# 1275468127/Medical-SAM2

Measured on AMD Instinct MI355X. Metric: slices/sec @1024^2 (Hiera-S), higher is better.
Workload: dtype bf16; 1 GPU; configs[1]: sam2_hiera_s 2D (train_2d SAM2 sub-sequence, forward), b=4 x 1024x1024 per GPU, 16-entry memory bank with 4 sampled memories per slice, one click per slice; forward_image -> memory_attention -> prompt encoder -> mask decoder -> memory encoder; hip_graph=True, weights=random name-keyed init

## Files before the change

### include/msam2_hip.h

```cpp
#ifndef MSAM2_HIP_H
#define MSAM2_HIP_H

#include <stddef.h>
#include <stdint.h>

#ifdef __cplusplus
extern "C" {
#endif

const char* msam2_last_error(void);

int msam2_version(void);

int msam2_operand_is_fp16(void);

int msam2_graph_begin(void* stream);

int msam2_graph_end(void* stream, void** graph_exec_out);

int msam2_graph_launch(void* graph_exec, void* stream);

int msam2_graph_destroy(void* graph_exec);

int msam2_event_create(void** ev);
// ... 47 lines not shown
int msam2_attention_kv64_dyn_fwd(const void* q, const int64_t* q_strides, const void* k, const int64_t* k_strides, const void* v, const int64_t* v_strides, void* o, const int64_t* o_strides, int64_t B, int64_t H, int64_t Lq, int64_t Lk, const void* key_count_dev, float scale, int splits, void* workspace, size_t workspace_bytes, void* stream);

int msam2_attention_kv64_dyn_partial(const void* q, const int64_t* q_strides, const void* k, const int64_t* k_strides, const void* v, const int64_t* v_strides, int64_t B, int64_t H, int64_t Lq, int64_t Lk, const void* key_count_dev, float scale, int splits, int split_begin, int split_count, void* workspace, size_t workspace_bytes, void* stream);

int msam2_window_attention_fwd(const void* q, int64_t q_token_stride, int64_t q_head_stride, int64_t hq, int64_t wq, int64_t ws_q, const void* k, const void* v, int64_t kv_token_stride, int64_t kv_head_stride, int64_t hk, int64_t wk, int64_t ws_k, const float* kpad, const float* vpad, void* o, int64_t o_token_stride, int64_t o_head_stride, int64_t B, int64_t H, int64_t D, float scale, void* stream);

int msam2_attention_small_fwd(const void* q, int64_t q_bs, int64_t q_ts, const void* k, int64_t k_bs, int64_t k_ts, const void* v, int64_t v_bs, int64_t v_ts, void* o, int64_t o_bs, int64_t o_ts, int64_t B, int64_t H, int64_t Lq, int64_t Lk, int64_t D, float scale, void* stream);

int msam2_attention_fewq_keysplit_splits(int64_t B, int64_t H);

int msam2_attention_fewq_keysplit(const void* q, int64_t q_bs, int64_t q_ts, const void* k, int64_t k_bs, int64_t k_ts, const void* v, int64_t v_bs, int64_t v_ts, float* part, int64_t B, int64_t H, int64_t Lq, int64_t Lk, int64_t D, int64_t splits, float scale, void* stream);

int msam2_window_qkv_attention_supported(int64_t dim, int64_t dim_out, int64_t heads, int64_t ws, int pool, int64_t H, int64_t W);

int msam2_window_qkv_attention_fwd(const void* xn, const void* w, const float* bias, void* o, int64_t B, int64_t H, int64_t W, int64_t dim, int64_t heads, int64_t ws, int pool, float scale, void* stream);

size_t msam2_attention_bwd_workspace_bytes(int64_t B, int64_t H, int64_t Lq, int64_t D);

int msam2_attention_bwd(const void* q, const int64_t* q_strides, const void* k, const int64_t* k_strides, const void* v, const int64_t* v_strides, const void* o, const int64_t* o_strides, const float* lse, const float* d_o, const int64_t* do_strides, float* dq, const int64_t* dq_strides, float* dk, const int64_t* dk_strides, float* dv, const int64_t* dv_strides, void* workspace, size_t workspace_bytes, int64_t B, int64_t H, int64_t Lq, int64_t Lk, int64_t D, float scale, void* stream);

int msam2_attention_bwd_dropout(const void* q, const int64_t* q_strides, const void* k, const int64_t* k_strides, const void* v, const int64_t* v_strides, const void* o, const int64_t* o_strides, const float* lse, const float* d_o, const int64_t* do_strides, float* dq, const int64_t* dq_strides, float* dk, const int64_t* dk_strides, float* dv, const int64_t* dv_strides, void* workspace, size_t workspace_bytes, int64_t B, int64_t H, int64_t Lq, int64_t Lk, int64_t D, float scale, float p, uint64_t seed, uint64_t offset, const void* seed_dev, void* stream);

int msam2_layernorm(const void* x, int in_is_16bit, int64_t ldx, const float* weight, const float* bias, void* y, int out_is_16bit, int64_t ldy, int64_t rows, int64_t C, float eps, int act, void* stream);

int msam2_layernorm_dual(const float* x, int64_t ldx, const float* weight, const float* bias, float* y, int64_t ldy, void* y16, int64_t ldy16, int64_t rows, int64_t C, float eps, void* stream);

int msam2_add_cast(const void* a, int a_is_16bit, int64_t a_s0, int64_t a_s1, const void* b, int b_is_16bit, int64_t b_s0, int64_t b_s1, float alpha, void* out, int out_is_16bit, int64_t D0, int64_t D1, int64_t C, void* stream);

int msam2_maxpool2x2(const void* x, int in_is_16bit, int64_t ldx, void* y, int out_is_16bit, int64_t ldy, int64_t B, int64_t H, int64_t W, int64_t C, void* stream);

// ... 249 lines not shown
```

### medical-sam2_amd/_lib.py

```python
from __future__ import annotations

import ctypes
import os
import subprocess

_HERE = os.path.dirname(os.path.abspath(__file__))
LIB_PATH = os.environ.get("MSAM2_LIB_PATH") or os.path.join(_HERE, "libmsam2_hip.so")

c_p = ctypes.c_void_p
c_i = ctypes.c_int
c_l = ctypes.c_int64
c_f = ctypes.c_float
c_z = ctypes.c_size_t
c_d = ctypes.c_double

SIGNATURES = {
    "msam2_version": (c_i, []),
    "msam2_last_error": (ctypes.c_char_p, []),
    "msam2_operand_is_fp16": (c_i, []),
    "msam2_gemm": (c_i, [c_p, c_l, c_p, c_l, c_p, c_p, c_p, c_l, c_i, c_l, c_p, c_l, c_i, c_l, c_l, c_l, c_i, c_p]),
    "msam2_gemm_pool2x2": (c_i, [c_p, c_l, c_p, c_l, c_p, c_p, c_l, c_l, c_l, c_l, c_l, c_l, c_p]),
    "msam2_gemm_qkv_pool2x2": (c_i, [c_p, c_l, c_p, c_l, c_p, c_p, c_l, c_p, c_l, c_l, c_l, c_l, c_l, c_l, c_l, c_p]),
    "msam2_gemm_tokens": (c_i, [c_p, c_l, c_p, c_l, c_p, c_l, c_p, c_p, c_l, c_p, c_l, c_i, c_l, c_l, c_l, c_i, c_p]),
    "msam2_gemm_rope": (c_i, [c_p, c_l, c_p, c_l, c_p, c_p, c_l, c_l, c_l, c_l, c_p, c_p, c_l, c_l, c_l, c_l, c_l, c_p]),
# ... 15 lines not shown
    "msam2_attention_workspace_bytes": (c_z, [c_l, c_l, c_l, c_l, c_i]),
    "msam2_attention_fwd": (c_i, [c_p, c_p, c_p, c_p, c_p, c_p, c_p, c_p, c_l, c_l, c_l, c_l, c_l, c_f, c_i, c_p, c_z, c_p]),
    "msam2_attention_fwd_lse": (c_i, [c_p, c_p, c_p, c_p, c_p, c_p, c_p, c_p, c_l, c_l, c_l, c_l, c_l, c_f, c_i, c_p, c_z, c_p, c_p]),
    "msam2_attention_fwd_lse_dropout": (c_i, [c_p, c_p, c_p, c_p, c_p, c_p, c_p, c_p, c_l, c_l, c_l, c_l, c_l, c_f, c_i, c_p, c_z, c_p, c_f,
                                              ctypes.c_uint64, ctypes.c_uint64, c_p, c_p]),
    "msam2_attention_kv64_fwd": (c_i, [c_p, c_p, c_p, c_p, c_p, c_p, c_p, c_p, c_l, c_l, c_l, c_l, c_f, c_i, c_p, c_z, c_p]),
    "msam2_attention_kv64_partial": (c_i, [c_p, c_p, c_p, c_p, c_p, c_p, c_l, c_l, c_l, c_l, c_f, c_i, c_i, c_i, c_p, c_z, c_p]),
    "msam2_attention_kv64_dyn_fwd": (c_i, [c_p, c_p, c_p, c_p, c_p, c_p, c_p, c_p, c_l, c_l, c_l, c_l, c_p, c_f, c_i, c_p, c_z, c_p]),
    "msam2_attention_kv64_dyn_partial": (c_i, [c_p, c_p, c_p, c_p, c_p, c_p, c_l, c_l, c_l, c_l, c_p, c_f, c_i, c_i, c_i, c_p, c_z, c_p]),
    "msam2_attention_effective_splits": (c_i, [c_l, c_i]),
    "msam2_attention_merge": (c_i, [c_p, c_p, c_l, c_l, c_l, c_l, c_l, c_i, c_p, c_z, c_p]),
    "msam2_window_attention_fwd": (c_i, [c_p, c_l, c_l, c_l, c_l, c_l, c_p, c_p, c_l, c_l, c_l, c_l, c_l, c_p, c_p, c_p, c_l, c_l,
                                         c_l, c_l, c_l, c_f, c_p]),
    "msam2_window_qkv_attention_supported": (c_i, [c_l, c_l, c_l, c_l, c_i, c_l, c_l]),
    "msam2_window_qkv_attention_fwd": (c_i, [c_p, c_p, c_p, c_p, c_l, c_l, c_l, c_l, c_l, c_l, c_i, c_f, c_p]),
    "msam2_attention_small_fwd": (c_i, [c_p, c_l, c_l, c_p, c_l, c_l, c_p, c_l, c_l, c_p, c_l, c_l, c_l, c_l, c_l, c_l, c_l, c_f,
                                        c_p]),
    "msam2_add_cast": (c_i, [c_p, c_i, c_l, c_l, c_p, c_i, c_l, c_l, c_f, c_p, c_i, c_l, c_l, c_l, c_p]),
    "msam2_maxpool2x2": (c_i, [c_p, c_i, c_l, c_p, c_i, c_l, c_l, c_l, c_l, c_l, c_p]),
    "msam2_upsample2x_add": (c_i, [c_p, c_p, c_l, c_l, c_l, c_l, c_p]),
    "msam2_rope_table": (c_i, [c_p, c_p, c_l, c_l, c_f, c_p]),
    "msam2_rope_inplace": (c_i, [c_p, c_l, c_l, c_l, c_l, c_l, c_l, c_l, c_p, c_p, c_p]),
    "msam2_bilinear_upsample": (c_i, [c_p, c_p, c_l, c_l, c_l, c_l, c_l, c_p]),
    "msam2_sine_pos_2d": (c_i, [c_p, c_l, c_l, c_l, c_f, c_p]),
    "msam2_fourier_pe_grid": (c_i, [c_p, c_p, c_l, c_l, c_l, c_p]),
    "msam2_hiera_pos_embed": (c_i, [c_p, c_p, c_p, c_l, c_l, c_l, c_l, c_l, c_l, c_p]),
    "msam2_im2col_patch7x7s4": (c_i, [c_p, c_p, c_l, c_l, c_p]),
    "msam2_patch_embed7x7s4": (c_i, [c_p, c_p, c_p, c_p, c_p, c_l, c_l, c_l, c_p]),
    "msam2_im2col3x3s2": (c_i, [c_p, c_p, c_l, c_l, c_l, c_l, c_l, c_p]),
    "msam2_conv3x3s2_ln_gelu": (c_i, [c_p, c_i, c_p, c_p, c_p, c_p, c_p, c_l, c_l, c_l, c_l, c_l, c_i, c_f, c_f, c_p]),
# ... 159 lines not shown
```

### medical-sam2_amd/csrc/attention.hip

```cpp
#include "common.h"
#ifdef MSAM2_STAMP
__device__ unsigned long long g_stamp[16];
__device__ unsigned long long g_wgtime[4096][4];
#define STAMP(var)                                                                     \
  do {                                                                                 \
    __builtin_amdgcn_sched_barrier(0);                                                 \
    asm volatile("s_memtime %0\n\ts_waitcnt lgkmcnt(0)" : "=s"(var)::"memory");         \
    __builtin_amdgcn_sched_barrier(0);                                                 \
  } while (0)
#define STAMP_DECL unsigned long long t0_ = 0, t1_ = 0, t2_ = 0, t3_ = 0, t4_ = 0, t5_ = 0, acc_[5] = {0, 0, 0, 0, 0}
#else
#define STAMP(var)
#define STAMP_DECL
#endif
#include <stdlib.h>
#include <type_traits>

#ifndef MSAM2_RESCALE_SLACK
#define MSAM2_RESCALE_SLACK 8.f
#endif

struct AttnParams {
  const op16 *q, *k, *v;
  op16* o;
  int64_t q_bs, q_hs, q_ts, k_bs, k_hs, k_ts, v_bs, v_hs, v_ts, o_bs, o_hs, o_ts;
  int B, H, Lq, Lk;
  float scale_log2;
  int win, ws_q, ws_k, hq, wq, hk, wk, nwy, nwx;
  const float *kpad, *vpad;
  int splits;
  int defer_merge;
  int split_begin, split_cnt;
  const int* lk_dev;
  op16* o_part;
  float* ml_part;
// ... 7 lines not shown
  static constexpr int KS = D * 2 + 16;
  static constexpr int VS = D * 2 + (((D * 2) % 128 == 64) ? 0 : 64);
  static constexpr int STAGE = BK * (KS + VS);
  static constexpr int LDS_BYTES = 2 * STAGE;
};


struct WgCoords {
  int x, y, z;
};
__device__ __forceinline__ WgCoords xcd_wg_coords() {
  const int gx = gridDim.x, gy = gridDim.y;
  const int nwg = gx * gy * gridDim.z;
  const int lid = xcd_tile_order(blockIdx.x + gx * (blockIdx.y + gy * blockIdx.z), nwg);
  return {lid % gx, (lid / gx) % gy, lid / (gx * gy)};
}

template <int DBLK>
__device__ __forceinline__ void softmax_move_reference(float mx, float& m_run, float& l_run, f32x16 (&o)[DBLK]) {
  const float m_new = fmaxf(m_run, mx);
  if (__any(m_new > m_run + MSAM2_RESCALE_SLACK)) {
    const float alpha = (m_run == -INFINITY) ? 0.f : __builtin_amdgcn_exp2f(m_run - m_new);
    l_run *= alpha;
#pragma unroll
    for (int d = 0; d < DBLK; ++d)
#pragma unroll
      for (int e = 0; e < 16; ++e) o[d][e] *= alpha;
    m_run = m_new;
  }
}

__device__ __forceinline__ int64_t win_token_offset(int t, int ws, int wy, int wx, int himg, int wimg, bool& valid) {
  const int ty = t / ws, tx = t - ty * ws;
  const int y = wy * ws + ty, x = wx * ws + tx;
  valid = (y < himg) && (x < wimg);
  return (int64_t)y * wimg + x;
}

template <int D, int NW, bool WIN>
__global__ __launch_bounds__(NW * 64, (WIN && NW == 4) ? 3 : 1) void attn_fwd_kernel(AttnParams p) {
  using C = AttnCfg<D>;
  constexpr int NT = NW * 64;
  constexpr int DSTEPS = D / 16;
  constexpr int DBLK = D / 32;
// ... 1551 lines not shown
  ws1_ = __builtin_amdgcn_s_memrealtime();
#endif
  if (wave * 32 >= p.Lq) return;

  f32x16 o[DBLK];
#pragma unroll
  for (int d = 0; d < DBLK; ++d)
#pragma unroll
    for (int e = 0; e < 16; ++e) o[d][e] = 0.f;
  float m_run = -INFINITY, l_run = 0.f;
  const int li = lane & 15;
  const int v_off = (4 * h + (li >> 2)) * RB + (16 * ((lane >> 4) & 1) + 4 * (li & 3)) * 2;
  const int ntiles = (p.Lk + BK - 1) / BK, nfull = p.Lk / BK;
  auto tile_step = [&](int tile, auto masked_tag) __attribute__((always_inline)) {
    constexpr bool MASKED = decltype(masked_tag)::value;
    const int key0 = tile * BK;
    const int krow = key0 + r;
    const unsigned char* kp = ksm + krow * RB;
    const int kx = (krow >> 2) & 3;
    f32x16 s;
#pragma unroll
    for (int e = 0; e < 16; ++e) s[e] = 0.f;
#pragma unroll
    for (int st = 0; st < DSTEPS; ++st) {
      const int c = 2 * st + h;
      const op16x8 kf = *reinterpret_cast<const op16x8*>(kp + (((c & ~3) | ((c & 3) ^ kx)) << 4));
      s = MSAM2_MFMA_32x32x16(kf, qf[st], s, 0, 0, 0);
    }
    float mx = -INFINITY;
#pragma unroll
    for (int e = 0; e < 16; ++e) {
      if constexpr (MASKED) {
        if (key0 + s_frag_key(e, h) >= p.Lk) s[e] = -INFINITY;
      }
      mx = fmaxf(mx, s[e]);
    }
    mx = half_max(mx) * p.scale_log2;
    softmax_move_reference(mx, m_run, l_run, o);
    float psum = 0.f;
    op16x8 pf[2];
    const float nm = -m_run;
#pragma unroll
    for (int e = 0; e < 16; ++e) {
      const float pe = __builtin_amdgcn_exp2f(__builtin_fmaf(s[e], p.scale_log2, nm));
      psum += pe;
      pf[e >> 3][e & 7] = f2op_fast(pe);
    }
    l_run += psum;
    const int nv = MASKED ? min(BK, lk8 - key0) : BK;
#pragma unroll
    for (int d = 0; d < DBLK; ++d) {
#pragma unroll
      for (int st = 0; st < 2; ++st) {
        const unsigned char* a0 = vsm + (key0 + 16 * st) * RB + v_off + d * 64;
        short4_t lo = {0, 0, 0, 0}, hi = {0, 0, 0, 0};
        if (!MASKED || 16 * st < nv) lo = __builtin_amdgcn_ds_read_tr16_b64_v4i16((short4_t __attribute__((address_space(3)))*)(a0));
        if (!MASKED || 16 * st + 8 < nv) hi = __builtin_amdgcn_ds_read_tr16_b64_v4i16((short4_t __attribute__((address_space(3)))*)(a0 + 8 * RB));
        short8_t vv8;
        vv8[0] = lo[0]; vv8[1] = lo[1]; vv8[2] = lo[2]; vv8[3] = lo[3];
        vv8[4] = hi[0]; vv8[5] = hi[1]; vv8[6] = hi[2]; vv8[7] = hi[3];
        o[d] = MSAM2_MFMA_32x32x16(__builtin_bit_cast(op16x8, vv8), pf[st], o[d], 0, 0, 0);
      }
    }
  };
  for (int tile = 0; tile < nfull; ++tile) tile_step(tile, std::false_type{});
  if (nfull < ntiles) tile_step(nfull, std::true_type{});
  const float l_tot = half_sum(l_run);
#ifdef MSAM2_STAMP
  ws2_ = __builtin_amdgcn_s_memrealtime();
#endif
  const float inv = 1.f / l_tot;
  if (qvalid) ATTN_STORE_O_ROWS(DBLK, p.o + (int64_t)b * p.o_bs + (int64_t)head * p.o_hs + qtok * p.o_ts, o, inv, h);
#ifdef MSAM2_STAMP
  wait_vmcnt<0>();
  ws3_ = __builtin_amdgcn_s_memrealtime();
  if (tid == 0) {
    const int wg = blockIdx.x + gridDim.x * blockIdx.y;
    if (wg < 4096) { g_wgtime[wg][0] = ws0_; g_wgtime[wg][1] = ws1_; g_wgtime[wg][2] = ws2_; g_wgtime[wg][3] = ws3_; }
// ... 679 lines not shown
```

### medical-sam2_amd/csrc/attn_winproj.hip

```cpp
#include "common.h"
#include <stdlib.h>

struct WinProjParams {
  const op16* xn;
  const op16* w;
  const float* bias;
  op16* o;
  int heads, H, W, nwx, nw;
  int n_units;
  float scale_log2;
};

__device__ __forceinline__ float quad_max(float v) {
  const int a = __builtin_amdgcn_mov_dpp(__builtin_bit_cast(int, v), 0xB1, 0xF, 0xF, true);
  v = fmaxf(v, __builtin_bit_cast(float, a));
  const int b = __builtin_amdgcn_mov_dpp(__builtin_bit_cast(int, v), 0x4E, 0xF, 0xF, true);
  return fmaxf(v, __builtin_bit_cast(float, b));
}

template <int DIM, int NB, bool QUADMAX>
__device__ __forceinline__ void winproj_T(const unsigned char* slab, const float* bias, const op16x8 (&xf)[NB][DIM / 16], int r, int h,
                                          op16x8 (&out)[NB][3][2]) {
  constexpr int KS = DIM / 16, RB = DIM * 2;
#pragma unroll
// ... 187 lines not shown
          f32x16 o[1];
#pragma unroll
          for (int e = 0; e < 16; ++e) o[0][e] = 0.f;
#pragma unroll
          for (int kb = 0; kb < NB; ++kb)
#pragma unroll
            for (int st = 0; st < 2; ++st) o[0] = MSAM2_MFMA_32x32x16(vf[kb][st], pf[qb][kb][st], o[0], 0, 0, 0);
          if (do_store) ATTN_STORE_O_ROWS(1, p.o + otok[qb] * (heads * D) + head * D + db * 32, o, inv[qb], h);
        }
      }
    }
  }
#endif
}

extern "C" int msam2_window_qkv_attention_supported(int64_t dim, int64_t dim_out, int64_t heads, int64_t ws, int pool, int64_t H,
                                                    int64_t W) {
  if (heads <= 0 || dim_out != heads * 96 || H <= 0 || W <= 0) return 0;
  if (!(ws == 8 || ws == 4) || H % ws || W % ws) return 0;
  if (pool && (H % 2 || W % 2)) return 0;
  if (ws == 4 && ((H / 4) * (W / 4)) % 2) return 0;
  if (dim == 96) return ws == 8 && heads <= 2;
  if (dim == 192) return ws == 4 && heads <= 8;
  return 0;
}

template <int DIM, int WS, bool POOL, bool STREAM>
static int launch_winproj(const WinProjParams& p, hipStream_t s) {
  constexpr int NWV = 8, SLAB = 96 * DIM * 2;
  const int lds = (STREAM ? 2 : 3 * p.heads) * SLAB + 3 * p.heads * 96 * 4;
  ensure_dyn_lds<attn_winproj_kernel<DIM, WS, POOL, STREAM, NWV>>(160 * 1024);
  const int n_pass = (p.n_units + NWV - 1) / NWV;
  hipLaunchKernelGGL((attn_winproj_kernel<DIM, WS, POOL, STREAM, NWV>), dim3((unsigned)min(256, n_pass)), dim3(NWV * 64), lds, s, p);
  return msam2_check_launch("window_qkv_attention_fwd");
}

extern "C" int msam2_window_qkv_attention_fwd(const void* xn, const void* w, const float* bias, void* o, int64_t B, int64_t H, int64_t W,
                                              int64_t dim, int64_t heads, int64_t ws, int pool, float scale, void* stream) {
  MSAM2_REQUIRE(xn && w && bias && o, "window_qkv_attention: null tensor");
  MSAM2_REQUIRE(B > 0 && H > 0 && W > 0 && heads > 0, "window_qkv_attention: empty problem");
  MSAM2_REQUIRE(msam2_window_qkv_attention_supported(dim, heads * 96, heads, ws, pool, H, W),
                "window_qkv_attention: dim %lld, %lld heads, window %lld, pool %d on %lld x %lld tokens is not built", (long long)dim,
                (long long)heads, (long long)ws, pool, (long long)H, (long long)W);
  MSAM2_REQUIRE((((uintptr_t)xn | (uintptr_t)w | (uintptr_t)bias) & 15) == 0 && ((uintptr_t)o & 7) == 0, "window_qkv_attention: 16-byte aligned tensors");
  MSAM2_REQUIRE(scale > 0.f, "window_qkv_attention: scale must be positive");
  const int64_t nw = (H / ws) * (W / ws), units = ws == 8 ? B * nw : B * nw / 2;
  MSAM2_REQUIRE(B * nw < (1ll << 30), "window_qkv_attention: too many windows");
  WinProjParams p = {(const op16*)xn, (const op16*)w, bias, (op16*)o, (int)heads, (int)H, (int)W, (int)(W / ws), (int)nw, (int)units,
                     scale * 1.4426950408889634f};
  hipStream_t s = (hipStream_t)stream;
  if (dim == 96) return pool ? launch_winproj<96, 8, true, false>(p, s) : launch_winproj<96, 8, false, false>(p, s);
  return pool ? launch_winproj<192, 4, true, true>(p, s) : launch_winproj<192, 4, false, true>(p, s);
}
```

### medical-sam2_amd/csrc/common.h

```cpp
#pragma once
#include <hip/hip_runtime.h>
#include <stdint.h>

#if defined(MSAM2_OPERAND_BF16)
typedef __bf16 op16;
#define MSAM2_OPERAND_IS_FP16 0
#define MSAM2_MFMA_32x32x16 __builtin_amdgcn_mfma_f32_32x32x16_bf16
#else
typedef _Float16 op16;
#define MSAM2_OPERAND_IS_FP16 1
#define MSAM2_MFMA_32x32x16 __builtin_amdgcn_mfma_f32_32x32x16_f16
#endif
typedef __attribute__((ext_vector_type(8))) op16 op16x8;
typedef __attribute__((ext_vector_type(4))) op16 op16x4;
typedef __attribute__((ext_vector_type(2))) op16 op16x2;
typedef __attribute__((ext_vector_type(4))) short short4_t;
typedef __attribute__((ext_vector_type(8))) short short8_t;
typedef __attribute__((ext_vector_type(16))) float f32x16;
typedef __attribute__((ext_vector_type(4))) float f32x4;

#define MSAM2_OK 0
#define MSAM2_ERR_ARG -1
#define MSAM2_ERR_LAUNCH -2

// ... 137 lines not shown
template <int ROW_BYTES_>
struct DmaImage {
  static constexpr int ROW_BYTES = ROW_BYTES_;
  static_assert(ROW_BYTES == 128 || ROW_BYTES == 64, "two images exist: 128-byte rows, slot c ^ ((r >> 1) & 7); 64-byte rows, c ^ ((r >> 2) & 3)");
  static constexpr int CPR = ROW_BYTES / 16;
  static constexpr int PIECE_ROWS = 1024 / ROW_BYTES;
  __device__ __forceinline__ static int swz(int r) { return (r >> (ROW_BYTES == 128 ? 1 : 2)) & (CPR - 1); }
  __device__ __forceinline__ static int piece_row(int piece, int lane) { return piece * PIECE_ROWS + (lane >> (ROW_BYTES == 128 ? 3 : 2)); }
  __device__ __forceinline__ static int src_chunk(int r, int lane) { return (lane & (CPR - 1)) ^ swz(r); }
};
typedef DmaImage<128> Img128;
typedef DmaImage<64> Img64;

template <int RB>
__device__ __forceinline__ int mlp_swz(int c, int r) {
  if constexpr (RB == 192) return (c & ~3) | ((c & 3) ^ ((r >> 2) & 3));
  else return (c & ~7) | ((c & 7) ^ ((r >> 1) & 7));
}

__device__ __forceinline__ constexpr int s_frag_key(int e, int h) { return (e & 3) + 8 * (e >> 2) + 4 * h; }

#define ATTN_STORE_O_ROWS(DBLK, dst, o, inv, h)                                           \
  do {                                                                                \
    op16* const dst_ = (dst);                                                         \
    _Pragma("unroll") for (int d_ = 0; d_ < DBLK; ++d_)                               \
      _Pragma("unroll") for (int g_ = 0; g_ < 4; ++g_) {                              \
        op16x4 w_;                                                                    \
        _Pragma("unroll") for (int e_ = 0; e_ < 4; ++e_) w_[e_] = f2op((o)[d_][4 * g_ + e_] * (inv)); \
        *reinterpret_cast<op16x4*>(dst_ + d_ * 32 + 8 * g_ + 4 * (h)) = w_;           \
      }                                                                               \
  } while (0)
// ... 280 lines not shown
```

### medical-sam2_amd/modeling/encoder.py

```python
from __future__ import annotations

from typing import List, Optional, Tuple

import torch
import torch.nn as nn

from .. import ops
from .common import OP16, F32, WeightCache, nchw_view, to_bf16, tokens_of, v_f32, w_bf16
from .position import PositionEmbeddingSine


import os as _os
_POOL_GEMM = _os.environ.get("MSAM2_NO_POOL_GEMM") is None
_QPOOL_GEMM = _os.environ.get("MSAM2_NO_QPOOL_GEMM") is None
_FUSED_MLP = _os.environ.get("MSAM2_NO_FUSED_MLP") is None
_FUSED_QKV_ATTN = _os.environ.get("MSAM2_NO_FUSED_QKV_ATTN") is None
_FUSED_PATCH = _os.environ.get("MSAM2_NO_FUSED_PATCH") is None
_FUSED_GEMM_LN = _os.environ.get("MSAM2_NO_FUSED_GEMM_LN") is None
_FUSED_GEMM_LN_K = frozenset(int(k) for k in _os.environ.get("MSAM2_FUSED_GEMM_LN_K", "384,1536").split(",") if k.strip())
_FUSED_MLP_LN = _os.environ.get("MSAM2_NO_FUSED_MLP_LN") is None
_FUSED_MLP_LN_MIN_TOKENS = 1024
_FUSED_PROJ_MLP = _os.environ.get("MSAM2_NO_FUSED_PROJ_MLP") is None
_FUSED_PROJ_MLP_DIMS = frozenset(int(k) for k in _os.environ.get("MSAM2_FUSED_PROJ_MLP_DIMS", "96,192").split(",") if k.strip())
_FUSED_PROJ_MLP_NEXT_LN_DIMS = frozenset(int(k) for k in _os.environ.get("MSAM2_FUSED_PROJ_MLP_NEXT_LN_DIMS", "").split(",") if k.strip())
_TWO_LAUNCH = 0


class two_launch_qkv_attention:

    def __enter__(self):
        global _TWO_LAUNCH
# ... 188 lines not shown
        scale = 1.0 / (D ** 0.5)
        if xn is None:
            xn = ops.layernorm(t, v_f32(wc, "n1w", self.norm1.weight), v_f32(wc, "n1b", self.norm1.bias), 1e-6)
        pool = self.q_stride is not None
        if self.dim != dim_out:
            if _POOL_GEMM and pool and B * H * W >= 256 and H % 2 == 0 and W % 2 == 0:
                shortcut = ops.gemm_pool2x2(xn, w_bf16(wc, "pw", self.proj.weight), v_f32(wc, "pb", self.proj.bias), B, H, W)
            else:
                shortcut = ops.gemm(xn, w_bf16(wc, "pw", self.proj.weight), v_f32(wc, "pb", self.proj.bias), out_dtype=F32)
                if pool:
                    shortcut = ops.maxpool2x2(shortcut, B, H, W)
        else:
            shortcut = t
        Hq, Wq = (H // 2, W // 2) if pool else (H, W)
        attn_in_one_kernel = (fused_qkv_attn and _FUSED_QKV_ATTN and self.window_size > 0 and Dp == D
                              and ops.window_qkv_attention_supported(self.dim, dim_out, heads, self.window_size, pool, H, W))
        if attn_in_one_kernel:
            o = ops.window_qkv_attention(xn, qkv_w, qkv_b, B, H, W, heads, self.window_size, pool, scale)
        else:
            if _POOL_GEMM and _QPOOL_GEMM and pool and B * H * W >= 256 and H % 2 == 0 and W % 2 == 0 and width % 32 == 0:
                qkv, qp = ops.gemm_qkv_pool2x2(xn, qkv_w, qkv_b, B, H, W, width)
            else:
                qkv = ops.gemm(xn, qkv_w, qkv_b)
                qp = ops.maxpool2x2(qkv[:, :width], B, H, W) if pool else None
            if self.window_size > 0:
                o = ops.window_attention(qkv, B, H, W, heads, self.window_size, qkv_b, q_pooled=qp, scale=scale)
            else:
                v5 = qkv.view(B, H * W, 3, heads, Dp)
                q = (qp.view(B, Hq * Wq, heads, Dp) if pool else v5[:, :, 0]).permute(0, 2, 1, 3)
                o = ops.attention(q, v5[:, :, 1].permute(0, 2, 1, 3), v5[:, :, 2].permute(0, 2, 1, 3), scale=scale)
# ... 176 lines not shown
```

### medical-sam2_amd/ops.py

```python
from __future__ import annotations

import ctypes
import math
from typing import Optional, Tuple

import torch

from ._lib import check, lib

OP16 = torch.float16 if lib().msam2_operand_is_fp16() else torch.bfloat16

F32 = torch.float32
ACT_NONE, ACT_GELU, ACT_RELU, ACT_SIGMOID = 0, 1, 2, 3


def _stream() -> int:
    return torch.cuda.current_stream().cuda_stream


def _p(t: Optional[torch.Tensor]):
    return None if t is None else t.data_ptr()


def _is_bf16(t: torch.Tensor) -> int:
# ... 461 lines not shown
def window_qkv_attention_supported(dim: int, dim_out: int, heads: int, ws: int, pool: bool, H: int, W: int) -> bool:
    return bool(lib().msam2_window_qkv_attention_supported(dim, dim_out, heads, ws, int(bool(pool)), H, W))


def window_qkv_attention(xn: torch.Tensor, w: torch.Tensor, bias: torch.Tensor, B: int, H: int, W: int, heads: int, ws: int,
                         pool: bool = False, scale: Optional[float] = None) -> torch.Tensor:
    _req(xn.dim() == 2 and w.dim() == 2 and xn.shape[0] == B * H * W and xn.shape[1] == w.shape[1] and w.shape[0] == 3 * heads * 96,
         "window_qkv_attention shapes")
    _req(xn.dtype == OP16 and w.dtype == OP16 and xn.is_contiguous() and w.is_contiguous(), "window_qkv_attention operands: 16-bit, contiguous")
    _req(bias.dtype == F32 and bias.is_contiguous() and bias.numel() == w.shape[0], "window_qkv_attention: bias is fp32 [3*heads*96]")
    hq, wq = (H // 2, W // 2) if pool else (H, W)
    o = torch.empty(B * hq * wq, heads * 96, dtype=OP16, device=xn.device)
    check(lib().msam2_window_qkv_attention_fwd(_p(xn), _p(w), _p(bias), _p(o), B, H, W, xn.shape[1], heads, ws, int(bool(pool)),
                                               scale if scale is not None else 1.0 / math.sqrt(96), _stream()))
    return o


def attention_small(q: torch.Tensor, k: torch.Tensor, v: torch.Tensor, heads: int, out: Optional[torch.Tensor] = None) -> torch.Tensor:
    B, Lq, C = q.shape
    Lk = k.shape[1]
    D = C // heads
    for t in (q, k, v):
        _req(t.dtype == OP16 and t.stride(2) == 1, "attention_small tensors must be 16-bit (ops.OP16), channel-contiguous")
    o = out if out is not None else torch.empty(B, Lq, C, dtype=OP16, device=q.device)
    _req(o.dtype == OP16 and o.shape == (B, Lq, C) and o.stride(2) == 1, "attention_small: out is 16-bit [B,Lq,C] with contiguous channels")
    check(lib().msam2_attention_small_fwd(_p(q), q.stride(0), q.stride(1), _p(k), k.stride(0), k.stride(1), _p(v), v.stride(0),
                                          v.stride(1), _p(o), o.stride(0), o.stride(1), B, heads, Lq, Lk, D,
                                          1.0 / math.sqrt(D), _stream()))
    return o

# ... 1233 lines not shown
```

Before: 793.1 slices/s.

## Fuse QKV projection and 14x14 window attention for dim-384 Hiera stage

Adds a fused kernel for the dim-384, 4-head, window-14 Hiera stage. It streams QKV weight pieces through double-buffered LDS, projects K/V/Q per window and head, and runs flash-style attention in the same kernel, so the QKV tensor is never written to global memory. Work units are ordered by cost and include partial edge windows, whose padded keys are filled with the bias values. The shared tile step is moved into a macro header, and the encoder enables the path by default when H*W >= 1024. The trade-off is recomputing K/V projections per head inside a one-block-per-CU kernel with large LDS use, which limits occupancy.

```diff
diff --git a/include/msam2_hip.h b/include/msam2_hip.h
--- a/include/msam2_hip.h
+++ b/include/msam2_hip.h
@@ -85,6 +85,8 @@
 int msam2_window_qkv_attention_supported(int64_t dim, int64_t dim_out, int64_t heads, int64_t ws, int pool, int64_t H, int64_t W);
 
 int msam2_window_qkv_attention_fwd(const void* xn, const void* w, const float* bias, void* o, int64_t B, int64_t H, int64_t W, int64_t dim, int64_t heads, int64_t ws, int pool, float scale, void* stream);
+
+int msam2_window_qkv_attention_units(int64_t B, int64_t H, int64_t W, int64_t heads, int32_t* out, int64_t cap);
 
 size_t msam2_attention_bwd_workspace_bytes(int64_t B, int64_t H, int64_t Lq, int64_t D);
 
diff --git a/medical-sam2_amd/_lib.py b/medical-sam2_amd/_lib.py
--- a/medical-sam2_amd/_lib.py
+++ b/medical-sam2_amd/_lib.py
@@ -53,6 +53,7 @@
                                          c_l, c_l, c_l, c_f, c_p]),
     "msam2_window_qkv_attention_supported": (c_i, [c_l, c_l, c_l, c_l, c_i, c_l, c_l]),
     "msam2_window_qkv_attention_fwd": (c_i, [c_p, c_p, c_p, c_p, c_l, c_l, c_l, c_l, c_l, c_l, c_i, c_f, c_p]),
+    "msam2_window_qkv_attention_units": (c_i, [c_l, c_l, c_l, c_l, c_p, c_l]),
     "msam2_attention_small_fwd": (c_i, [c_p, c_l, c_l, c_p, c_l, c_l, c_p, c_l, c_l, c_p, c_l, c_l, c_l, c_l, c_l, c_l, c_l, c_f,
                                         c_p]),
     "msam2_add_cast": (c_i, [c_p, c_i, c_l, c_l, c_p, c_i, c_l, c_l, c_f, c_p, c_i, c_l, c_l, c_l, c_p]),
diff --git a/medical-sam2_amd/csrc/attention.hip b/medical-sam2_amd/csrc/attention.hip
--- a/medical-sam2_amd/csrc/attention.hip
+++ b/medical-sam2_amd/csrc/attention.hip
@@ -16,9 +16,7 @@
 #include <stdlib.h>
 #include <type_traits>
 
-#ifndef MSAM2_RESCALE_SLACK
-#define MSAM2_RESCALE_SLACK 8.f
-#endif
+#include "attn_wintile.h"
 
 struct AttnParams {
   const op16 *q, *k, *v;
@@ -56,20 +54,6 @@
   const int nwg = gx * gy * gridDim.z;
   const int lid = xcd_tile_order(blockIdx.x + gx * (blockIdx.y + gy * blockIdx.z), nwg);
   return {lid % gx, (lid / gx) % gy, lid / (gx * gy)};
-}
-
-template <int DBLK>
-__device__ __forceinline__ void softmax_move_reference(float mx, float& m_run, float& l_run, f32x16 (&o)[DBLK]) {
-  const float m_new = fmaxf(m_run, mx);
-  if (__any(m_new > m_run + MSAM2_RESCALE_SLACK)) {
-    const float alpha = (m_run == -INFINITY) ? 0.f : __builtin_amdgcn_exp2f(m_run - m_new);
-    l_run *= alpha;
-#pragma unroll
-    for (int d = 0; d < DBLK; ++d)
-#pragma unroll
-      for (int e = 0; e < 16; ++e) o[d][e] *= alpha;
-    m_run = m_new;
-  }
 }
 
 __device__ __forceinline__ int64_t win_token_offset(int t, int ws, int wy, int wx, int himg, int wimg, bool& valid) {
@@ -1651,54 +1635,7 @@
   const int ntiles = (p.Lk + BK - 1) / BK, nfull = p.Lk / BK;
   auto tile_step = [&](int tile, auto masked_tag) __attribute__((always_inline)) {
     constexpr bool MASKED = decltype(masked_tag)::value;
-    const int key0 = tile * BK;
-    const int krow = key0 + r;
-    const unsigned char* kp = ksm + krow * RB;
-    const int kx = (krow >> 2) & 3;
-    f32x16 s;
-#pragma unroll
-    for (int e = 0; e < 16; ++e) s[e] = 0.f;
-#pragma unroll
-    for (int st = 0; st < DSTEPS; ++st) {
-      const int c = 2 * st + h;
-      const op16x8 kf = *reinterpret_cast<const op16x8*>(kp + (((c & ~3) | ((c & 3) ^ kx)) << 4));
-      s = MSAM2_MFMA_32x32x16(kf, qf[st], s, 0, 0, 0);
-    }
-    float mx = -INFINITY;
-#pragma unroll
-    for (int e = 0; e < 16; ++e) {
-      if constexpr (MASKED) {
-        if (key0 + s_frag_key(e, h) >= p.Lk) s[e] = -INFINITY;
-      }
-      mx = fmaxf(mx, s[e]);
-    }
-    mx = half_max(mx) * p.scale_log2;
-    softmax_move_reference(mx, m_run, l_run, o);
-    float psum = 0.f;
-    op16x8 pf[2];
-    const float nm = -m_run;
-#pragma unroll
-    for (int e = 0; e < 16; ++e) {
-      const float pe = __builtin_amdgcn_exp2f(__builtin_fmaf(s[e], p.scale_log2, nm));
-      psum += pe;
-      pf[e >> 3][e & 7] = f2op_fast(pe);
-    }
-    l_run += psum;
-    const int nv = MASKED ? min(BK, lk8 - key0) : BK;
-#pragma unroll
-    for (int d = 0; d < DBLK; ++d) {
-#pragma unroll
-      for (int st = 0; st < 2; ++st) {
-        const unsigned char* a0 = vsm + (key0 + 16 * st) * RB + v_off + d * 64;
-        short4_t lo = {0, 0, 0, 0}, hi = {0, 0, 0, 0};
-        if (!MASKED || 16 * st < nv) lo = __builtin_amdgcn_ds_read_tr16_b64_v4i16((short4_t __attribute__((address_space(3)))*)(a0));
-        if (!MASKED || 16 * st + 8 < nv) hi = __builtin_amdgcn_ds_read_tr16_b64_v4i16((short4_t __attribute__((address_space(3)))*)(a0 + 8 * RB));
-        short8_t vv8;
-        vv8[0] = lo[0]; vv8[1] = lo[1]; vv8[2] = lo[2]; vv8[3] = lo[3];
-        vv8[4] = hi[0]; vv8[5] = hi[1]; vv8[6] = hi[2]; vv8[7] = hi[3];
-        o[d] = MSAM2_MFMA_32x32x16(__builtin_bit_cast(op16x8, vv8), pf[st], o[d], 0, 0, 0);
-      }
-    }
+    ATTN_WIN_TILE_STEP(tile, MASKED, p.Lk, p.scale_log2);
   };
   for (int tile = 0; tile < nfull; ++tile) tile_step(tile, std::false_type{});
   if (nfull < ntiles) tile_step(nfull, std::true_type{});
diff --git a/medical-sam2_amd/csrc/attn_winproj.hip b/medical-sam2_amd/csrc/attn_winproj.hip
--- a/medical-sam2_amd/csrc/attn_winproj.hip
+++ b/medical-sam2_amd/csrc/attn_winproj.hip
@@ -1,4 +1,5 @@
 #include "common.h"
+#include "attn_wintile.h"
 #include <stdlib.h>
 
 struct WinProjParams {
@@ -225,9 +226,249 @@
 #endif
 }
 
+struct Win384Units {
+  int B, H, W, heads;
+  int fy, fx, ry, rx;
+  int kind[4], win[4], end[4];
+  int n_units;
+};
+
+struct Win384Unit {
+  int b, wy, wx, head, vh, vw;
+};
+
+static inline Win384Units win384_units(int64_t B, int64_t H, int64_t W, int64_t heads) {
+  Win384Units u = {};
+  u.B = (int)B; u.H = (int)H; u.W = (int)W; u.heads = (int)heads;
+  u.fy = (int)(H / 14); u.fx = (int)(W / 14); u.ry = (int)(H % 14); u.rx = (int)(W % 14);
+  const int win[4] = {u.fy * u.fx, u.rx ? u.fy : 0, u.ry ? u.fx : 0, (u.rx && u.ry) ? 1 : 0};
+  const int tok[4] = {196, 14 * u.rx, 14 * u.ry, u.ry * u.rx};
+  int order[4] = {0, 1, 2, 3};
+  auto cost = [&](int k) { return win[k] ? (tok[k] + 31) / 32 : 0; };
+  for (int i = 1; i < 4; ++i)
+    for (int j = i; j > 0 && cost(order[j]) > cost(order[j - 1]); --j) { const int t = order[j]; order[j] = order[j - 1]; order[j - 1] = t; }
+  int run = 0;
+  for (int c = 0; c < 4; ++c) {
+    u.kind[c] = order[c]; u.win[c] = win[order[c]];
+    run += u.B * u.win[c] * u.heads;
+    u.end[c] = run;
+  }
+  u.n_units = run;
+  return u;
+}
+
+__host__ __device__ __forceinline__ Win384Unit win384_unit(const Win384Units& u, int j) {
+  int c = 0;
+  while (c < 3 && j >= u.end[c]) ++c;
+  if (c) j -= u.end[c - 1];
+  const int kind = u.kind[c], nw = u.win[c];
+  const int wi = j % nw, b = (j / nw) % u.B, head = j / (nw * u.B);
+  switch (kind) {
+    case 0: return {b, wi / u.fx, wi % u.fx, head, 14, 14};
+    case 1: return {b, wi, u.fx, head, 14, u.rx};
+    case 2: return {b, u.fy, wi, head, u.ry, 14};
+    default: return {b, u.fy, u.fx, head, u.ry, u.rx};
+  }
+}
+
+struct Win384Params {
+  const op16* xn;
+  const op16* w;
+  const float* bias;
+  op16* o;
+  Win384Units u;
+  float scale_log2;
+};
+
+#ifndef WIN384_AG
+#define WIN384_AG 4
+#endif
+constexpr int WIN384_WAVES = 7, WIN384_PIECE_BYTES = 32 * 768, WIN384_LK = 196, WIN384_LK8 = 200;
+constexpr int WIN384_LDS = 2 * WIN384_PIECE_BYTES + (WIN384_LK + WIN384_LK8) * 192 + 3 * 4 * 96 * 4;
+
+__global__ __launch_bounds__(WIN384_WAVES * 64, 1) void attn_winproj384_kernel(Win384Params p) {
+#if defined(__HIP_DEVICE_COMPILE__)
+  constexpr int D = 96, DIM = 384, KS = DIM / 16, WRB = DIM * 2, CPR = DIM / 8, HEADS = 4, WS = 14, NWV = WIN384_WAVES;
+  constexpr int RB = D * 2, DSTEPS = D / 16, DBLK = D / 32, BK = 32, LK = WIN384_LK, lk8 = WIN384_LK8;
+  constexpr int AG = WIN384_AG, PIECE = WIN384_PIECE_BYTES, DMAS = PIECE / 1024, PW = (DMAS + NWV - 1) / NWV, STEPS = 9;
+  extern __shared__ __attribute__((aligned(1024))) unsigned char smem[];
+  unsigned char* const ksm = smem + 2 * PIECE;
+  unsigned char* const vsm = ksm + LK * RB;
+  float* const bsm = reinterpret_cast<float*>(vsm + lk8 * RB);
+  const int tid = threadIdx.x;
+  const int wave = __builtin_amdgcn_readfirstlane(tid >> 6), lane = tid & 63;
+  const int r = lane & 31, h = lane >> 5;
+  for (int i = tid; i < 3 * HEADS * D; i += NWV * 64) bsm[i] = p.bias[i];
+  if (tid < (lk8 - LK) * RB / 16) *reinterpret_cast<uint4*>(vsm + LK * RB + tid * 16) = make_uint4(0, 0, 0, 0);
+
+  const auto w_rsrc = raw_rsrc(p.w, 3 * HEADS * D * WRB);
+  unsigned off[PW];
+#pragma unroll
+  for (int j = 0; j < PW; ++j) {
+    const int f = min(j * NWV + wave, DMAS - 1) * 64 + lane, row = f / CPR, c = f % CPR;
+    off[j] = (unsigned)(row * WRB + mlp_swz<WRB>(c, row) * 16);
+  }
+  auto issue = [&](int head, int s, int slot) {
+    const unsigned soff = (unsigned)((((s / 3 == 2 ? 0 : s / 3 + 1) * HEADS + head) * D + (s % 3) * 32) * WRB);
+    unsigned char* d = smem + slot * PIECE;
+#pragma unroll
+    for (int j = 0; j < PW; ++j)
+      if (j * NWV + wave < DMAS) glds16_asm(w_rsrc, d + (j * NWV + wave) * 1024, off[j], soff);
+  };
+
+  const int n_units = p.u.n_units;
+  issue(win384_unit(p.u, blockIdx.x).head, 0, 0);
+  __syncthreads();
+  int g_step = 0;
+  const int swap_r = (r & ~12) | ((r & 4) << 1) | ((r & 8) >> 1);
+  auto chunk_offsets = [&](int row, int (&aoff)[8]) {
+#pragma unroll
+    for (int k = 0; k < 8; ++k) aoff[k] = mlp_swz<WRB>(2 * k + h, row) << 4;
+  };
+  const int li = lane & 15;
+  const int v_off = (4 * h + (li >> 2)) * RB + (16 * ((lane >> 4) & 1) + 4 * (li & 3)) * 2;
+
+#pragma unroll 1
+  for (int j = blockIdx.x; j < n_units; j += gridDim.x) {
+    const Win384Unit un = win384_unit(p.u, j);
+    const int head = un.head, nvalid = un.vh * un.vw;
+    const int jn = j + (int)gridDim.x;
+    const int next_head = jn < n_units ? win384_unit(p.u, jn).head : -1;
+    auto piece_ptr = [&](int s) -> const unsigned char* {
+      const int slot = g_step & 1;
+      wait_vmcnt<0>();
+      __syncthreads();
+      if (s + 1 < STEPS) issue(head, s + 1, slot ^ 1);
+      else if (next_head >= 0) issue(next_head, 0, slot ^ 1);
+      ++g_step;
+      return smem + slot * PIECE;
+    };
+
+    const bool wave_on = wave * 32 < nvalid;
+    const int v = wave * 32 + r;
+    const bool valid = v < nvalid;
+    const int vc = min(v, nvalid - 1), ty = vc / un.vw, tx = vc - ty * un.vw;
+    const int key = ty * WS + tx;
+    const int64_t tok = ((int64_t)un.b * p.u.H + un.wy * WS + ty) * p.u.W + un.wx * WS + tx;
+    auto pad_rows = [&]() {
+      for (int c = tid; c < LK * (RB / 16); c += NWV * 64) {
+        const int pk = c / (RB / 16), cc = c - pk * (RB / 16), py = pk / WS, px = pk - py * WS;
+        if (py >= un.vh || px >= un.vw) {
+          op16x8 a, bb;
+#pragma unroll
+          for (int e = 0; e < 8; ++e) {
+            a[e] = f2op(bsm[(HEADS + head) * D + cc * 8 + e]);
+            bb[e] = f2op(bsm[(2 * HEADS + head) * D + cc * 8 + e]);
+          }
+          *reinterpret_cast<op16x8*>(ksm + pk * RB + (((cc & ~3) | ((cc & 3) ^ ((pk >> 2) & 3))) << 4)) = a;
+          *reinterpret_cast<op16x8*>(vsm + pk * RB + (cc << 4)) = bb;
+        }
+      }
+    };
+    if (!wave_on) {
+#pragma unroll 1
+      for (int s = 0; s < STEPS; ++s) {
+        piece_ptr(s);
+        if (s == 0 && nvalid < LK) pad_rows();
+      }
+      continue;
+    }
+    op16x8 xf[KS];
+    {
+      const op16* xr = p.xn + tok * DIM;
+#pragma unroll
+      for (int k = 0; k < KS; ++k) xf[k] = __builtin_bit_cast(op16x8, *reinterpret_cast<const uint4*>(xr + 16 * k + 8 * h));
+    }
+    auto project = [&](const unsigned char* pc, int row, const int (&aoff)[8]) -> f32x16 {
+      const unsigned char* pr = pc + row * WRB;
+      f32x16 acc;
+#pragma unroll
+      for (int e = 0; e < 16; ++e) acc[e] = 0.f;
+      op16x8 a[2][AG];
+#pragma unroll
+      for (int i = 0; i < AG; ++i) a[0][i] = *reinterpret_cast<const op16x8*>(pr + aoff[i]);
+#pragma unroll
+      for (int g = 0; g < KS / AG; ++g) {
+        if (g + 1 < KS / AG) {
+#pragma unroll
+          for (int i = 0; i < AG; ++i) {
+            const int k = AG * (g + 1) + i;
+            a[(g + 1) & 1][i] = *reinterpret_cast<const op16x8*>(pr + aoff[k & 7] + 256 * (k >> 3));
+          }
+        }
+#pragma unroll
+        for (int i = 0; i < AG; ++i) acc = MSAM2_MFMA_32x32x16(a[g & 1][i], xf[AG * g + i], acc, 0, 0, 0);
+        __builtin_amdgcn_sched_barrier(0);
+      }
+      return acc;
+    };
+
+    int aoff_k[8];
+    chunk_offsets(r, aoff_k);
+#pragma unroll 1
+    for (int s = 0; s < 6; ++s) {
+      const int isv = s / 3, db = s % 3;
+      const unsigned char* pc = piece_ptr(s);
+      if (s == 0 && nvalid < LK) pad_rows();
+      {
+        const f32x16 acc = project(pc, r, aoff_k);
+        const float* bp = bsm + ((1 + isv) * HEADS + head) * D + db * 32 + 4 * h;
+        if (valid) {
+#pragma unroll
+          for (int g = 0; g < 4; ++g) {
+            const f32x4 bv = *reinterpret_cast<const f32x4*>(bp + 8 * g);
+            op16x4 w4;
+#pragma unroll
+            for (int e = 0; e < 4; ++e) w4[e] = f2op(acc[4 * g + e] + bv[e]);
+            const int cc = 4 * db + g;
+            if (isv) *reinterpret_cast<op16x4*>(vsm + key * RB + (cc << 4) + 8 * h) = w4;
+            else *reinterpret_cast<op16x4*>(ksm + key * RB + (((cc & ~3) | ((cc & 3) ^ ((key >> 2) & 3))) << 4) + 8 * h) = w4;
+          }
+        }
+      }
+    }
+    op16x8 qf[DSTEPS];
+    const unsigned qmask = valid ? 0xffffffffu : 0u;
+    int aoff_q[8];
+    chunk_offsets(swap_r, aoff_q);
+#pragma unroll
+    for (int db = 0; db < DBLK; ++db) {
+      const unsigned char* pc = piece_ptr(6 + db);
+      {
+        const f32x16 acc = project(pc, swap_r, aoff_q);
+        const float* bp = bsm + head * D + db * 32 + 8 * h;
+#pragma unroll
+        for (int st = 0; st < 2; ++st) {
+          const f32x4 b0 = *reinterpret_cast<const f32x4*>(bp + 16 * st), b1 = *reinterpret_cast<const f32x4*>(bp + 16 * st + 4);
+#pragma unroll
+          for (int e = 0; e < 4; ++e) {
+            qf[2 * db + st][e] = f2op(acc[8 * st + e] + b0[e]);
+            qf[2 * db + st][4 + e] = f2op(acc[8 * st + 4 + e] + b1[e]);
+          }
+          uint4 qu = __builtin_bit_cast(uint4, qf[2 * db + st]);
+          qu.x &= qmask; qu.y &= qmask; qu.z &= qmask; qu.w &= qmask;
+          qf[2 * db + st] = __builtin_bit_cast(op16x8, qu);
+        }
+      }
+    }
+
+    __builtin_amdgcn_sched_barrier(0);
+    f32x16 o[DBLK];
+    zero_acc(o);
+    float m_run = -INFINITY, l_run = 0.f;
+#pragma unroll 1
+    for (int tile = 0; tile < LK / BK; ++tile) ATTN_WIN_TILE_STEP(tile, false, LK, p.scale_log2);
+    ATTN_WIN_TILE_STEP(LK / BK, true, LK, p.scale_log2);
+    const float inv = 1.f / half_sum(l_run);
+    if (valid) ATTN_STORE_O_ROWS(DBLK, p.o + tok * (HEADS * D) + head * D, o, inv, h);
+  }
+#endif
+}
+
 extern "C" int msam2_window_qkv_attention_supported(int64_t dim, int64_t dim_out, int64_t heads, int64_t ws, int pool, int64_t H,
                                                     int64_t W) {
   if (heads <= 0 || dim_out != heads * 96 || H <= 0 || W <= 0) return 0;
+  if (ws == 14) return dim == 384 && heads == 4 && !pool;
   if (!(ws == 8 || ws == 4) || H % ws || W % ws) return 0;
   if (pool && (H % 2 || W % 2)) return 0;
   if (ws == 4 && ((H / 4) * (W / 4)) % 2) return 0;
@@ -255,11 +496,31 @@
                 (long long)heads, (long long)ws, pool, (long long)H, (long long)W);
   MSAM2_REQUIRE((((uintptr_t)xn | (uintptr_t)w | (uintptr_t)bias) & 15) == 0 && ((uintptr_t)o & 7) == 0, "window_qkv_attention: 16-byte aligned tensors");
   MSAM2_REQUIRE(scale > 0.f, "window_qkv_attention: scale must be positive");
+  hipStream_t s = (hipStream_t)stream;
+  if (ws == 14) {
+    MSAM2_REQUIRE(B * ((H + 13) / 14) * ((W + 13) / 14) * heads < (1ll << 30) && B * H * W < (1ll << 31), "window_qkv_attention: too many windows");
+    Win384Params q = {(const op16*)xn, (const op16*)w, bias, (op16*)o, win384_units(B, H, W, heads), scale * 1.4426950408889634f};
+    ensure_dyn_lds<attn_winproj384_kernel>(160 * 1024);
+    hipLaunchKernelGGL(attn_winproj384_kernel, dim3((unsigned)min(256, q.u.n_units)), dim3(WIN384_WAVES * 64), WIN384_LDS, s, q);
+    return msam2_check_launch("window_qkv_attention_fwd(384)");
+  }
   const int64_t nw = (H / ws) * (W / ws), units = ws == 8 ? B * nw : B * nw / 2;
   MSAM2_REQUIRE(B * nw < (1ll << 30), "window_qkv_attention: too many windows");
   WinProjParams p = {(const op16*)xn, (const op16*)w, bias, (op16*)o, (int)heads, (int)H, (int)W, (int)(W / ws), (int)nw, (int)units,
                      scale * 1.4426950408889634f};
-  hipStream_t s = (hipStream_t)stream;
   if (dim == 96) return pool ? launch_winproj<96, 8, true, false>(p, s) : launch_winproj<96, 8, false, false>(p, s);
   return pool ? launch_winproj<192, 4, true, true>(p, s) : launch_winproj<192, 4, false, true>(p, s);
 }
+
+extern "C" int msam2_window_qkv_attention_units(int64_t B, int64_t H, int64_t W, int64_t heads, int32_t* out, int64_t cap) {
+  MSAM2_REQUIRE(B > 0 && msam2_window_qkv_attention_supported(heads * 96, heads * 96, heads, 14, 0, H, W), "window_qkv_attention_units: form not built");
+  MSAM2_REQUIRE(B * ((H + 13) / 14) * ((W + 13) / 14) * heads < (1ll << 30), "window_qkv_attention_units: too many windows");
+  MSAM2_REQUIRE(cap >= 0 && (out || cap == 0), "window_qkv_attention_units: null list");
+  const Win384Units u = win384_units(B, H, W, heads);
+  for (int j = 0; j < u.n_units && j < cap; ++j) {
+    const Win384Unit un = win384_unit(u, j);
+    const int row[5] = {un.b, un.wy, un.wx, un.head, (un.vh * un.vw + 31) / 32};
+    for (int i = 0; i < 5; ++i) out[5 * j + i] = row[i];
+  }
+  return u.n_units;
+}
diff --git a/medical-sam2_amd/csrc/attn_wintile.h b/medical-sam2_amd/csrc/attn_wintile.h
--- /dev/null
+++ b/medical-sam2_amd/csrc/attn_wintile.h
@@ -0,0 +1,67 @@
+#pragma once
+#include "common.h"
+
+#ifndef MSAM2_RESCALE_SLACK
+#define MSAM2_RESCALE_SLACK 8.f
+#endif
+
+template <int DBLK>
+__device__ __forceinline__ void softmax_move_reference(float mx, float& m_run, float& l_run, f32x16 (&o)[DBLK]) {
+  const float m_new = fmaxf(m_run, mx);
+  if (__any(m_new > m_run + MSAM2_RESCALE_SLACK)) {
+    const float alpha = (m_run == -INFINITY) ? 0.f : __builtin_amdgcn_exp2f(m_run - m_new);
+    l_run *= alpha;
+#pragma unroll
+    for (int d = 0; d < DBLK; ++d)
+#pragma unroll
+      for (int e = 0; e < 16; ++e) o[d][e] *= alpha;
+    m_run = m_new;
+  }
+}
+
+#define ATTN_WIN_TILE_STEP(tile, MASKED, Lk, scale_log2)                                                                                  \
+  do {                                                                                                                                    \
+    const int key0 = (tile) * BK;                                                                                                         \
+    const int krow = key0 + r;                                \
+    const unsigned char* kp = ksm + krow * RB;                                                                                            \
+    const int kx = (krow >> 2) & 3;                                                                                                       \
+    f32x16 s;                                                                                                                             \
+    _Pragma("unroll") for (int e = 0; e < 16; ++e) s[e] = 0.f;                                                                            \
+    _Pragma("unroll") for (int st = 0; st < DSTEPS; ++st) {                                                                               \
+      const int c = 2 * st + h;                                                                                                           \
+      const op16x8 kf = *reinterpret_cast<const op16x8*>(kp + (((c & ~3) | ((c & 3) ^ kx)) << 4));                                        \
+      s = MSAM2_MFMA_32x32x16(kf, qf[st], s, 0, 0, 0);                                                                                    \
+    }                                                                                                                                     \
+    float mx = -INFINITY;                                                                                                                 \
+    _Pragma("unroll") for (int e = 0; e < 16; ++e) {                                                                                      \
+      if constexpr (MASKED) {                                                                                                             \
+        if (key0 + s_frag_key(e, h) >= (Lk)) s[e] = -INFINITY;                                                                            \
+      }                                                                                                                                   \
+      mx = fmaxf(mx, s[e]);                                                                                                               \
+    }                                                                                                                                     \
+    mx = half_max(mx) * (scale_log2);                                                                \
+    softmax_move_reference(mx, m_run, l_run, o);                                                                                          \
+    float psum = 0.f;                                                                                                                     \
+    op16x8 pf[2];                                                                                                                         \
+    const float nm = -m_run;                                                                 \
+    _Pragma("unroll") for (int e = 0; e < 16; ++e) {                                                                                      \
+      const float pe = __builtin_amdgcn_exp2f(__builtin_fmaf(s[e], (scale_log2), nm));                                                    \
+      psum += pe;                                                                                                                         \
+      pf[e >> 3][e & 7] = f2op_fast(pe);                                                                                                  \
+    }                                                                                                                                     \
+    l_run += psum;                                                                                                                        \
+    const int nv = MASKED ? min(BK, lk8 - key0) : BK;                          \
+    _Pragma("unroll") for (int d = 0; d < DBLK; ++d) {                                                                                    \
+      _Pragma("unroll") for (int st = 0; st < 2; ++st) {                                                                                  \
+                         \
+        const unsigned char* a0 = vsm + (key0 + 16 * st) * RB + v_off + d * 64;                                                           \
+        short4_t lo = {0, 0, 0, 0}, hi = {0, 0, 0, 0};                                                                                    \
+        if (!MASKED || 16 * st < nv) lo = __builtin_amdgcn_ds_read_tr16_b64_v4i16((short4_t __attribute__((address_space(3)))*)(a0));     \
+        if (!MASKED || 16 * st + 8 < nv) hi = __builtin_amdgcn_ds_read_tr16_b64_v4i16((short4_t __attribute__((address_space(3)))*)(a0 + 8 * RB)); \
+        short8_t vv8;                                                                                                                     \
+        vv8[0] = lo[0]; vv8[1] = lo[1]; vv8[2] = lo[2]; vv8[3] = lo[3];                                                                   \
+        vv8[4] = hi[0]; vv8[5] = hi[1]; vv8[6] = hi[2]; vv8[7] = hi[3];                                                                   \
+        o[d] = MSAM2_MFMA_32x32x16(__builtin_bit_cast(op16x8, vv8), pf[st], o[d], 0, 0, 0);                                               \
+      }                                                                                                                                   \
+    }                                                                                                                                     \
+  } while (0)
diff --git a/medical-sam2_amd/csrc/common.h b/medical-sam2_amd/csrc/common.h
--- a/medical-sam2_amd/csrc/common.h
+++ b/medical-sam2_amd/csrc/common.h
@@ -175,7 +175,8 @@
 
 template <int RB>
 __device__ __forceinline__ int mlp_swz(int c, int r) {
-  if constexpr (RB == 192) return (c & ~3) | ((c & 3) ^ ((r >> 2) & 3));
+  if constexpr (RB == 768) return c ^ (r & 15);
+  else if constexpr (RB == 192) return (c & ~3) | ((c & 3) ^ ((r >> 2) & 3));
   else return (c & ~7) | ((c & 7) ^ ((r >> 1) & 7));
 }
 
diff --git a/medical-sam2_amd/modeling/encoder.py b/medical-sam2_amd/modeling/encoder.py
--- a/medical-sam2_amd/modeling/encoder.py
+++ b/medical-sam2_amd/modeling/encoder.py
@@ -15,6 +15,8 @@
 _QPOOL_GEMM = _os.environ.get("MSAM2_NO_QPOOL_GEMM") is None
 _FUSED_MLP = _os.environ.get("MSAM2_NO_FUSED_MLP") is None
 _FUSED_QKV_ATTN = _os.environ.get("MSAM2_NO_FUSED_QKV_ATTN") is None
+_FUSED_QKV_ATTN_384 = _os.environ.get("MSAM2_NO_FUSED_QKV_ATTN_384") is None
+_FUSED_QKV_ATTN_384_MIN_TOKENS = 1024
 _FUSED_PATCH = _os.environ.get("MSAM2_NO_FUSED_PATCH") is None
 _FUSED_GEMM_LN = _os.environ.get("MSAM2_NO_FUSED_GEMM_LN") is None
 _FUSED_GEMM_LN_K = frozenset(int(k) for k in _os.environ.get("MSAM2_FUSED_GEMM_LN_K", "384,1536").split(",") if k.strip())
@@ -233,6 +235,7 @@
             shortcut = t
         Hq, Wq = (H // 2, W // 2) if pool else (H, W)
         attn_in_one_kernel = (fused_qkv_attn and _FUSED_QKV_ATTN and self.window_size > 0 and Dp == D
+                              and (self.dim != 384 or (_FUSED_QKV_ATTN_384 and H * W >= _FUSED_QKV_ATTN_384_MIN_TOKENS))
                               and ops.window_qkv_attention_supported(self.dim, dim_out, heads, self.window_size, pool, H, W))
         if attn_in_one_kernel:
             o = ops.window_qkv_attention(xn, qkv_w, qkv_b, B, H, W, heads, self.window_size, pool, scale)
diff --git a/medical-sam2_amd/ops.py b/medical-sam2_amd/ops.py
--- a/medical-sam2_amd/ops.py
+++ b/medical-sam2_amd/ops.py
@@ -499,6 +499,14 @@
     check(lib().msam2_window_qkv_attention_fwd(_p(xn), _p(w), _p(bias), _p(o), B, H, W, xn.shape[1], heads, ws, int(bool(pool)),
                                                scale if scale is not None else 1.0 / math.sqrt(96), _stream()))
     return o
+
+
+def window_qkv_attention_units(B: int, H: int, W: int, heads: int = 4) -> torch.Tensor:
+    n = lib().msam2_window_qkv_attention_units(B, H, W, heads, None, 0)
+    check(min(n, 0))
+    out = torch.empty(n, 5, dtype=torch.int32)
+    check(min(lib().msam2_window_qkv_attention_units(B, H, W, heads, _p(out), n), 0))
+    return out
 
 
 def attention_small(q: torch.Tensor, k: torch.Tensor, v: torch.Tensor, heads: int, out: Optional[torch.Tensor] = None) -> torch.Tensor:
```

New measurement: 794.3 slices/s (median of 6 runs). No clear change (+0.1%).
